# pmcbride/denoise-gan

Hardware: AMD Instinct MI355X
Metric: training images/sec, pix2pix 256x256 bs16/GPU (higher is better)
Workload: dtype fp32 (GEMMs fp16x3, operands 2^-22); 1 GPU; pix2pix train_step (train_pix2pix.py:33-71): G(x)+G(y) identity pass, D real+fake, GAN/L1/L2/TV/identity losses, D and G gradients, Keras Adam G and D; VGG19 content loss (seeded stand-in weights: ImageNet weights are a download); model=pix2pix U-Net G (54.4M) + PatchGAN D (2.77M), global_batch=16, batch_per_gpu=16, image_size=256, scale=1, parallelism=dp1, hip_graph=True, identity_pass=True

## Files before the change

### denoise-gan_amd/csrc/conv_tiles.h

```cpp
#pragma once

#define DG_TILES_FP32(X)                                                                         \
    X(0, 128, 128, 2, 2, 32, 2, 1, 2, 1.00)                                                      \
    X(1, 128, 64, 2, 2, 32, 2, 1, 2, 1.12)                                                       \
    X(2, 64, 128, 2, 2, 32, 2, 1, 2, 1.12)                                                       \
    X(3, 64, 64, 2, 2, 32, 2, 1, 3, 1.35)                                                        \
    X(4, 32, 128, 1, 4, 32, 2, 1, 3, 1.50)                                                       \
    X(5, 128, 128, 2, 2, 16, 3, 1, 3, 1.00)                                                      \
    X(6, 128, 64, 2, 2, 16, 3, 1, 3, 1.12)                                                       \
    X(7, 128, 32, 4, 1, 32, 2, 1, 3, 1.40)                                                       \
    X(8, 256, 32, 4, 1, 32, 2, 1, 2, 1.30)

#define DG_TILES_F16_BK 32
#define DG_TILES_X6(X)                                                                           \
    X(0, 128, 128, 2, 2, 16, 2, 3, 2, 1.00)                                                      \
    X(1, 128, 64, 2, 2, 16, 2, 3, 2, 1.15)                                                       \
    X(2, 64, 128, 2, 2, 16, 2, 3, 2, 1.15)                                                       \
    X(3, 64, 64, 2, 2, 16, 3, 3, 4, 1.40)                                                        \
    X(4, 256, 128, 4, 2, 16, 2, 3, 1, 1.00)                                                      \
    X(5, 128, 256, 2, 4, 16, 2, 3, 1, 0.90)                                                      \
    X(6, 128, 32, 4, 1, 16, 3, 3, 4, 1.45)

#ifndef DG_X3_NB0
#define DG_X3_NB0 2
#endif
#ifndef DG_X3_NB12
#define DG_X3_NB12 2
#endif
#define DG_TILES_X3(X)                                                                           \
    X(0, 128, 128, 2, 2, 32, 2, DG_X3_NB0, 2, 1.00)                                              \
    X(1, 128, 64, 2, 2, 32, 2, DG_X3_NB12, 3, 1.15)                                              \
    X(2, 64, 128, 2, 2, 32, 2, DG_X3_NB12, 3, 1.15)                                              \
    X(3, 64, 64, 2, 2, 32, 3, 3, 3, 1.40)                                                        \
    X(4, 256, 128, 4, 2, 32, 1, 2, 1, 1.00)                                                      \
    X(5, 128, 256, 2, 4, 32, 1, 2, 1, 0.90)                                                      \
    X(6, 128, 32, 4, 1, 32, 3, 3, 2, 1.45)
```

### denoise-gan_amd/csrc/conv_x6.hip

```cpp
#include "conv_x6.h"
#include "conv_tiles.h"
#include <algorithm>

namespace dg {

__global__ void __launch_bounds__(256)
k_split3(const float *__restrict__ src, int ld, long rows, int C, unsigned short *__restrict__ dst) {
    const int C8 = C >> 3;
    const long total = rows * C8;
    const bool vec = ((ld & 3) == 0) && ((((uintptr_t)src) & 15) == 0);
    for (long e = (long)blockIdx.x * blockDim.x + threadIdx.x; e < total; e += (long)gridDim.x * blockDim.x) {
        const long r = e / C8;
        const int c = (int)(e - r * C8) * 8;
        const float *sp = src + r * ld + c;
        f32x4 v0, v1;
        if (vec) {
            v0 = *reinterpret_cast<const f32x4 *>(sp);
            v1 = *reinterpret_cast<const f32x4 *>(sp + 4);
        } else {
            v0 = f32x4{sp[0], sp[1], sp[2], sp[3]};
            v1 = f32x4{sp[4], sp[5], sp[6], sp[7]};
        }
        unsigned h0, m0, l0, h1, m1, l1, h2, m2, l2, h3, m3, l3;
        split3(v0[0], v0[1], h0, m0, l0);
        split3(v0[2], v0[3], h1, m1, l1);
        split3(v1[0], v1[1], h2, m2, l2);
        split3(v1[2], v1[3], h3, m3, l3);
        unsigned short *d = dst + r * 3 * C + (c >> 4) * 48 + (c & 8);
        *reinterpret_cast<u32x4 *>(d) = u32x4{h0, h1, h2, h3};
        *reinterpret_cast<u32x4 *>(d + 16) = u32x4{m0, m1, m2, m3};
        *reinterpret_cast<u32x4 *>(d + 32) = u32x4{l0, l1, l2, l3};
    }
}

__global__ void __launch_bounds__(256)
k_split_f16(const float *__restrict__ src, int ld, long rows, int C, _Float16 *__restrict__ dst) {
    const int C8 = C >> 3;
    const long total = rows * C8;
    const bool vec = ((ld & 3) == 0) && ((((uintptr_t)src) & 15) == 0);
    for (long e = (long)blockIdx.x * blockDim.x + threadIdx.x; e < total; e += (long)gridDim.x * blockDim.x) {
        const long r = e / C8;
        const int c = (int)(e - r * C8) * 8;
        const float *sp = src + r * ld + c;
        f32x4 v0, v1;
        if (vec) {
            v0 = *reinterpret_cast<const f32x4 *>(sp);
            v1 = *reinterpret_cast<const f32x4 *>(sp + 4);
        } else {
            v0 = f32x4{sp[0], sp[1], sp[2], sp[3]};
            v1 = f32x4{sp[4], sp[5], sp[6], sp[7]};
        }
        f16x8 h;
#pragma unroll
        for (int q = 0; q < 4; ++q) { h[q] = (_Float16)v0[q]; h[4 + q] = (_Float16)v1[q]; }
        *reinterpret_cast<f16x8 *>(dst + r * C + c) = h;
    }
}

template <int MODE, int BM, int BN, int WGM, int WGN, int MINW, int NBUF = 3, int NI = 3>
__global__ void __launch_bounds__(64 * WGM * WGN, MINW)
k_conv_gemm_x6(const GemmArgs p) {
    static_assert(NBUF >= 2 && NBUF <= 4, "2 to 4 LDS buffers (1 to 3 K-tiles in flight)");
    static_assert(NI == 3 || NI == 2 || NI == 4, "bf16x6 (3 plane images), fp16 (2 chunk images), fp16x3 (4)");
    constexpr bool X6 = NI == 3;
    constexpr bool X3 = NI == 4;
    constexpr int BK = X6 ? 16 : 32;
    constexpr int GS = 16 * NI;
    constexpr int RM = X6 ? 3 : (X3 ? 2 : 1);
    constexpr bool A_KC = (MODE != MODE_WGRAD);
    constexpr bool B_KC = (MODE == MODE_DGRAD);
    constexpr int NT = 64 * WGM * WGN;
    constexpr int WTM = BM / WGM, WTN = BN / WGN;
    constexpr int TM = WTM / 16, TN = WTN / 16;
    constexpr int APL = BM * 32 + 96, BPL = BN * 32 + 96;
    constexpr int BUF = NI * (APL + BPL);
    constexpr int NW_ = WGM * WGN;
    static_assert(WGM * WGN == 4 || WGM * WGN == 8, "4 or 8 waves");
    static_assert(TM >= 1 && TN >= 1 && WTM % 16 == 0 && WTN % 16 == 0, "wave tile of 16x16 tiles");
    static_assert(BM % 32 == 0 && BN % 32 == 0 && BM <= 256 && BN <= 256, "tile");

    constexpr int STAGE = 16 * (WTN + 4);
    constexpr int BUF0 = BUF > NW_ * STAGE * 4 ? BUF : NW_ * STAGE * 4;
    __shared__ __attribute__((aligned(16))) char smem0[BUF0];
    __shared__ __attribute__((aligned(16))) char smem1[BUF];
    __shared__ __attribute__((aligned(16))) char smem2[NBUF >= 3 ? BUF : 16];
    __shared__ __attribute__((aligned(16))) char smem3[NBUF == 4 ? BUF : 16];

    const ConvGeom &g = p.g;
    const int tid = threadIdx.x;
    const int lane = tid & 63;
    const int wid = __builtin_amdgcn_readfirstlane(tid >> 6);
    const int wm = wid / WGN, wn = wid % WGN;
    const int l32 = lane & 31, h2 = lane >> 5;
    X3Pre x3s;
    if constexpr (X3) x3s = x3_pre(p);

    int zz, tile;
    xcd_remap(zz, tile);
    const int phase = zz / p.splits;
    const int split = zz - phase * p.splits;
    const int mt = tile / p.ntiles;
    const int nt = tile - mt * p.ntiles;
    const int m0 = mt * BM, n0 = nt * BN;

    int Mrows = p.M;
    PhaseInfo ph{};
    if constexpr (MODE == MODE_DGRAD) {
        ph = phase_info(g, phase, g.N);
        Mrows = ph.Mp;
        if (m0 >= Mrows) return;
    }
    const int kbeg = split * p.kchunk;
    const int kend = min(p.K, kbeg + p.kchunk);
    if (kbeg >= kend) return;
    const int nk = (kend - kbeg + BK - 1) / BK;

    constexpr int NW = WGM * WGN;
    constexpr int A_SL = NI * BM / 32, B_SL = NI * BN / 32;
    constexpr int A_NJ = (A_SL + NW - 1) / NW, B_NJ = (B_SL + NW - 1) / NW;
    struct Slot { int plane, r, c; bool live; };
    auto slot_of = [&](int d, bool kc, int X) __attribute__((always_inline)) {
        Slot sl; const int per = X / 32;
        sl.plane = d / per;
        const int pos = (d - sl.plane * per) * 1024 + 16 * lane;
        if (kc) {
            sl.r = pos >> 5;
            sl.c = (pos >> 4) & 1;
        } else {
            sl.r = pos / (2 * X);
            const int pdw = (pos - sl.r * 2 * X) >> 2;
            sl.c = 2 * (pdw ^ x6_rc_swz_cols(X, sl.r));
        }
        return sl;
    };
    Slot asl[A_NJ], bsl[B_NJ];
#pragma unroll
    for (int j = 0; j < A_NJ; ++j) {
        const int d = wid + NW * j;
        asl[j] = slot_of(d < A_SL ? d : 0, A_KC, BM);
        asl[j].live = d < A_SL;
    }
#pragma unroll
    for (int j = 0; j < B_NJ; ++j) {
        const int d = wid + NW * j;
        bsl[j] = slot_of(d < B_SL ? d : 0, B_KC, BN);
        bsl[j].live = d < B_SL;
    }
    constexpr bool A_ALL = (A_SL % NW) == 0, B_ALL = (B_SL % NW) == 0;
    constexpr int NMINE = A_NJ + B_NJ;

    int arow_n[A_NJ], arow_h[A_NJ], arow_w[A_NJ];
    int wg_i[A_NJ], wg_j[A_NJ], wg_ci[A_NJ];
#pragma unroll
    for (int j = 0; j < A_NJ; ++j) {
        arow_n[j] = -1; arow_h[j] = 0; arow_w[j] = 0; wg_i[j] = 0; wg_j[j] = 0; wg_ci[j] = 0;
        if constexpr (A_KC) {
            int m = m0 + asl[j].r;
            if (m < Mrows) {
                if constexpr (MODE == MODE_FWD) {
                    int wo = m % g.Wo; int t = m / g.Wo; int ho = t % g.Ho; int n = t / g.Ho;
                    arow_n[j] = n; arow_h[j] = ho * g.sh - g.pt; arow_w[j] = wo * g.sw - g.pl;
                } else {
                    int ww = m % ph.Wp; int t = m / ph.Wp; int hh = t % ph.Hp; int n = t / ph.Hp;
                    arow_n[j] = n;
                    arow_h[j] = hh + (ph.ph + g.pt - ph.i0h) / g.sh;
                    arow_w[j] = ww + (ph.pw + g.pl - ph.i0w) / g.sw;
                }
            }
        } else {
            int mc = m0 + asl[j].c;
            if (mc < p.M) {
                arow_n[j] = 0;
                int tap = mc / g.Ci; int ci = mc - tap * g.Ci; wg_i[j] = tap / g.kw; wg_j[j] = tap - wg_i[j] * g.kw;
                wg_ci[j] = X6 ? (ci >> 4) * 48 + 16 * asl[j].plane + (ci & 8)
                              : (X3 ? (ci >> 5) * 64 + 32 * (asl[j].plane >> 1) + (ci & 31) : ci);
            }
        }
    }

    const int TA = MODE == MODE_FWD ? g.kh : g.Th, TB = MODE == MODE_FWD ? g.kw : g.Tw;
    int wk_a = 0, wk_b = 0, wk_chunk = 0;
    if constexpr (MODE != MODE_WGRAD) {
        int kk = kbeg / BK; wk_chunk = kk / (TA * TB); int t = kk - wk_chunk * TA * TB;
        wk_a = t / TB; wk_b = t - wk_a * TB;
    }
    int abase[A_NJ], amask[A_NJ], bbase[B_NJ];
    bool bok[B_NJ];
    if constexpr (MODE != MODE_WGRAD) {
#pragma unroll
        for (int j = 0; j < A_NJ; ++j) {
            abase[j] = 0; amask[j] = 0;
            if (arow_n[j] < 0) continue;
            if constexpr (MODE == MODE_FWD) {
                abase[j] = (((arow_n[j] * g.H + arow_h[j]) * g.W + arow_w[j]) * (RM * p.lda) + 16 * asl[j].plane +
                            8 * asl[j].c) * 2;
                for (int a = 0; a < TA; ++a)
                    for (int b = 0; b < TB; ++b) {
                        const int hi = arow_h[j] + a, wi = arow_w[j] + b;
                        if ((unsigned)hi < (unsigned)g.H && (unsigned)wi < (unsigned)g.W) amask[j] |= 1 << (a * TB + b);
                    }
            } else {
                abase[j] = (((arow_n[j] * g.Ho + arow_h[j]) * g.Wo + arow_w[j]) * (RM * p.lda) + 16 * asl[j].plane +
                            8 * asl[j].c) * 2;
                for (int a = 0; a < TA; ++a)
                    for (int b = 0; b < TB; ++b) {
                        const int i = ph.i0h + a * g.sh, jj = ph.i0w + b * g.sw;
                        const int ho = arow_h[j] - a, wo = arow_w[j] - b;
                        if (i < g.kh && jj < g.kw && (unsigned)ho < (unsigned)g.Ho && (unsigned)wo < (unsigned)g.Wo)
                            amask[j] |= 1 << (a * TB + b);
                    }
            }
        }
#pragma unroll
        for (int j = 0; j < B_NJ; ++j) {
            if constexpr (MODE == MODE_FWD) {
                const int col = n0 + bsl[j].c;
                bok[j] = col < p.N;
                bbase[j] = X6 ? (bsl[j].r * (3 * p.ldb) + (col >> 4) * 48 + 16 * bsl[j].plane + (col & 8)) * 2
                         : X3 ? ((bsl[j].r + 16 * (bsl[j].plane & 1)) * (2 * p.ldb) + (col >> 4) * 32 +
                                 16 * (bsl[j].plane >> 1) + (col & 8)) * 2
                              : ((bsl[j].r + 16 * bsl[j].plane) * p.ldb + col) * 2;
            } else {
                const int ci = n0 + bsl[j].r;
                bok[j] = ci < p.N;
                bbase[j] = (ci * (RM * p.ldb) + 16 * bsl[j].plane + 8 * bsl[j].c) * 2;
            }
        }
    }
    auto walk_next = [&]() __attribute__((always_inline)) {
        const int nb = wk_b + 1;
        const bool wb = nb == TB;
        const int na = wk_a + (wb ? 1 : 0);
        const bool wa = na == TA;
        wk_b = wb ? 0 : nb;
        wk_a = wa ? 0 : na;
        wk_chunk += wa ? 1 : 0;
    };

    const rsrc4_t rA = make_rsrc4(p.A, p.a_bytes);
    const rsrc4_t rB = make_rsrc4(p.B, p.b_bytes);
    auto dma = [](rsrc4_t r, char *lds_base, unsigned off) __attribute__((always_inline)) { dma16(r, lds_base, off); };
    auto fdiv = [](unsigned n, unsigned mul, int shr) __attribute__((always_inline)) { return (__umulhi(n, mul) + n) >> shr; };

    auto issue_tile = [&](int k0, char *sm) __attribute__((always_inline)) {
        char *As = sm;
        char *Bs = As + NI * APL;
        int a_delta = 0, b_delta = 0, tap_bit = 0;
        bool b_tap_ok = true;
        if constexpr (MODE == MODE_FWD) {
            a_delta = ((wk_a * g.W + wk_b) * (RM * p.lda) + wk_chunk * GS) * 2;
            b_delta = (((wk_a * g.kw + wk_b) * g.Ci + wk_chunk * BK) * (RM * p.ldb)) * 2;
            tap_bit = wk_a * TB + wk_b;
        } else if constexpr (MODE == MODE_DGRAD) {
            a_delta = (wk_chunk * GS - (wk_a * g.Wo + wk_b) * (RM * p.lda)) * 2;
            const int i = ph.i0h + wk_a * g.sh, jj = ph.i0w + wk_b * g.sw;
            b_tap_ok = i < g.kh && jj < g.kw;
            b_delta = ((b_tap_ok ? (i * g.kw + jj) * g.Ci * (RM * p.ldb) : 0) + wk_chunk * GS) * 2;
            tap_bit = wk_a * TB + wk_b;
        }
        (void)a_delta; (void)b_delta; (void)tap_bit; (void)b_tap_ok;
        const bool live = MODE == MODE_WGRAD || k0 < kend;
#pragma unroll
        for (int j = 0; j < A_NJ; ++j) {
            const int d = asl[j].live ? wid + NW * j : 0, per = BM / 32;
            char *dst = As + asl[j].plane * APL + (d - asl[j].plane * per) * 1024;
            unsigned off;
            bool ok;
            if constexpr (MODE != MODE_WGRAD) {
                ok = (amask[j] >> tap_bit) & 1;
                off = (unsigned)(abase[j] + a_delta);
            } else {
                const unsigned pix = (unsigned)(k0 + asl[j].r + (X6 ? 0 : 16 * (X3 ? asl[j].plane & 1 : asl[j].plane)));
                const unsigned t = fdiv(pix, p.mg_wo, p.sh_wo); const int wo = (int)(pix - t * g.Wo);
                const unsigned n = fdiv(t, p.mg_ho, p.sh_ho); const int ho = (int)(t - n * g.Ho);
                const int hi = ho * g.sh - g.pt + wg_i[j], wi = wo * g.sw - g.pl + wg_j[j];
                ok = arow_n[j] >= 0 && (int)pix < kend && (unsigned)hi < (unsigned)g.H && (unsigned)wi < (unsigned)g.W;
                off = ((unsigned)(((int)n * g.H + hi) * g.W + wi) * (RM * p.lda) + wg_ci[j]) * 2u;
            }
            dma(rA, dst, ok && live ? off : DG_OOB);
        }
#pragma unroll
        for (int j = 0; j < B_NJ; ++j) {
            const int d = bsl[j].live ? wid + NW * j : 0, per = BN / 32;
            char *dst = Bs + bsl[j].plane * BPL + (d - bsl[j].plane * per) * 1024;
            unsigned off;
            bool ok;
            if constexpr (MODE == MODE_FWD) {
                ok = bok[j];
                off = (unsigned)(bbase[j] + b_delta);
            } else if constexpr (MODE == MODE_DGRAD) {
                ok = bok[j] && b_tap_ok;
                off = (unsigned)(bbase[j] + b_delta);
            } else {
                const int col = n0 + bsl[j].c;
                const int pix = k0 + bsl[j].r + (X6 ? 0 : 16 * (X3 ? bsl[j].plane & 1 : bsl[j].plane));
                ok = col < p.N && pix < kend;
                off = X6 ? ((unsigned)pix * (3 * p.ldb) + (col >> 4) * 48 + 16 * bsl[j].plane + (col & 8)) * 2u
                    : X3 ? ((unsigned)pix * (2 * p.ldb) + (col >> 5) * 64 + 32 * (bsl[j].plane >> 1) + (col & 31)) * 2u
                         : ((unsigned)pix * p.ldb + col) * 2u;
            }
            dma(rB, dst, ok && live ? off : DG_OOB);
        }
        if constexpr (MODE != MODE_WGRAD) walk_next();
    };
    auto barrier = []() __attribute__((always_inline)) {
        asm volatile("s_waitcnt lgkmcnt(0)" ::: "memory");
        __builtin_amdgcn_s_barrier();
        asm volatile("" ::: "memory");
    };

    f32x4 acc[TM][TN];
#pragma unroll
    for (int a = 0; a < TM; ++a)
#pragma unroll
        for (int b = 0; b < TN; ++b) acc[a][b] = f32x4{0.f, 0.f, 0.f, 0.f};

    auto frag = [&](const char *p0, const char *p1, int rc0, bool kc, bool is_a) __attribute__((always_inline)) {
        if (kc) return x6_kc_frag(p0, p1, rc0, lane);
        return is_a ? x6_rc_frag<BM>(p0, p1, rc0, lane) : x6_rc_frag<BN>(p0, p1, rc0, lane);
    };
    auto read_frags = [&](const char *sm, bf16x8 (&ahm)[TM], bf16x8 (&ahl)[TM], bf16x8 (&b1)[TN],
                          bf16x8 (&b2)[TN], bf16x8 (&b3)[TN]) __attribute__((always_inline)) {
        const char *A0 = sm, *A1 = sm + APL, *A2 = sm + (NI - 1) * APL;
        const char *B0 = sm + NI * APL, *B1 = B0 + BPL, *B2 = B0 + (NI - 1) * BPL;
#pragma unroll
        for (int a = 0; a < TM; ++a) {
            const int r0 = wm * WTM + a * 16;
            ahm[a] = frag(A0, A1, r0, A_KC, true);
            if constexpr (X6) ahl[a] = frag(A0, A2, r0, A_KC, true);
        }
#pragma unroll
        for (int b = 0; b < TN; ++b) {
            const int c0 = wn * WTN + b * 16;
            b1[b] = frag(B0, B1, c0, B_KC, false);
            if constexpr (X6) {
                b2[b] = frag(B1, B0, c0, B_KC, false);
                b3[b] = frag(B2, B0, c0, B_KC, false);
            }
        }
    };

    constexpr int AHEAD = NBUF - 1;
#if defined(DG_NO_MIDB)
    constexpr bool MIDB = false;
#elif defined(DG_MIDB_X3)
    constexpr bool MIDB = X3;
#else
    constexpr bool MIDB = true;
#endif
    constexpr int DIST = MIDB ? NBUF : AHEAD;
    auto ktile = [&](int kt, const char *cur, char *nxt) __attribute__((always_inline)) {
        if constexpr (X3) {
            f16x8 ah[TM], al[TM], bh[TN], bl[TN];
            const char *B0 = cur + 4 * APL;
#pragma unroll
            for (int a = 0; a < TM; ++a) {
                const int r0 = wm * WTM + a * 16;
                ah[a] = __builtin_bit_cast(f16x8, frag(cur, cur + APL, r0, A_KC, true));
                al[a] = __builtin_bit_cast(f16x8, frag(cur + 2 * APL, cur + 3 * APL, r0, A_KC, true));
            }
            constexpr int BH1 = B_KC ? 2 : 1, BL0 = B_KC ? 1 : 2;
#pragma unroll
            for (int b = 0; b < TN; ++b) {
                const int c0 = wn * WTN + b * 16;
                bh[b] = __builtin_bit_cast(f16x8, frag(B0, B0 + BH1 * BPL, c0, B_KC, false));
                bl[b] = __builtin_bit_cast(f16x8, frag(B0 + BL0 * BPL, B0 + 3 * BPL, c0, B_KC, false));
            }
            if constexpr (MIDB) {
                barrier();
                issue_tile(kbeg + (kt + DIST) * BK, const_cast<char *>(cur));
            } else {
                issue_tile(kbeg + (kt + AHEAD) * BK, nxt);
            }
#pragma unroll
            for (int a = 0; a < TM; ++a)
#pragma unroll
                for (int b = 0; b < TN; ++b)
                    acc[a][b] = __builtin_amdgcn_mfma_f32_16x16x32_f16(ah[a], bh[b], acc[a][b], 0, 0, 0);
#pragma unroll
            for (int a = 0; a < TM; ++a)
#pragma unroll
                for (int b = 0; b < TN; ++b)
                    acc[a][b] = __builtin_amdgcn_mfma_f32_16x16x32_f16(al[a], bh[b], acc[a][b], 0, 0, 0);
#pragma unroll
            for (int a = 0; a < TM; ++a)
#pragma unroll
                for (int b = 0; b < TN; ++b)
                    acc[a][b] = __builtin_amdgcn_mfma_f32_16x16x32_f16(ah[a], bl[b], acc[a][b], 0, 0, 0);
            wait_dma_c<(DIST - 1) * NMINE>();
            barrier();
            return;
        }
        bf16x8 ahm[TM], ahl[X6 ? TM : 1], b1[TN], b2[X6 ? TN : 1], b3[X6 ? TN : 1];
        if constexpr (X6) {
            read_frags(cur, ahm, ahl, b1, b2, b3);
        } else {
            bf16x8 dA[TM], dB[TN];
            read_frags(cur, ahm, dA, b1, dB, dB);
        }
        if constexpr (MIDB) {
            barrier();
            issue_tile(kbeg + (kt + DIST) * BK, const_cast<char *>(cur));
        } else {
            issue_tile(kbeg + (kt + AHEAD) * BK, nxt);
        }
        if constexpr (X6) {
#pragma unroll
            for (int a = 0; a < TM; ++a)
#pragma unroll
                for (int b = 0; b < TN; ++b)
                    acc[a][b] = __builtin_amdgcn_mfma_f32_16x16x32_bf16(ahm[a], b1[b], acc[a][b], 0, 0, 0);
#pragma unroll
            for (int a = 0; a < TM; ++a)
#pragma unroll
                for (int b = 0; b < TN; ++b)
                    acc[a][b] = __builtin_amdgcn_mfma_f32_16x16x32_bf16(ahm[a], b2[b], acc[a][b], 0, 0, 0);
#pragma unroll
            for (int a = 0; a < TM; ++a)
#pragma unroll
                for (int b = 0; b < TN; ++b)
                    acc[a][b] = __builtin_amdgcn_mfma_f32_16x16x32_bf16(ahl[a], b3[b], acc[a][b], 0, 0, 0);
        } else {
#pragma unroll
            for (int a = 0; a < TM; ++a)
#pragma unroll
                for (int b = 0; b < TN; ++b)
                    acc[a][b] = __builtin_amdgcn_mfma_f32_16x16x32_f16(__builtin_bit_cast(f16x8, ahm[a]),
                                                                       __builtin_bit_cast(f16x8, b1[b]), acc[a][b],
                                                                       0, 0, 0);
        }
        wait_dma_c<(DIST - 1) * NMINE>();
        barrier();
    };
    auto pipeline = [&](char *L0, char *L1, char *L2, char *L3) __attribute__((always_inline)) {
        issue_tile(kbeg, L0);
        if constexpr (DIST >= 2) issue_tile(kbeg + BK, L1);
        if constexpr (DIST >= 3) issue_tile(kbeg + 2 * BK, L2);
        if constexpr (DIST >= 4) issue_tile(kbeg + 3 * BK, L3);
        wait_dma_c<(DIST - 1) * NMINE>();
        barrier();
        int kt = 0;
        if constexpr (NBUF == 2) {
            for (; kt + 1 < nk; kt += 2) {
                ktile(kt, L0, L1);
                ktile(kt + 1, L1, L0);
            }
            if (kt < nk) ktile(kt, L0, L1);
        } else if constexpr (NBUF == 3) {
            for (; kt + 2 < nk; kt += 3) {
                ktile(kt, L0, L2);
                ktile(kt + 1, L1, L0);
                ktile(kt + 2, L2, L1);
            }
            if (kt < nk) ktile(kt, L0, L2);
            if (kt + 1 < nk) ktile(kt + 1, L1, L0);
        } else {
            for (; kt + 3 < nk; kt += 4) {
                ktile(kt, L0, L3);
                ktile(kt + 1, L1, L0);
                ktile(kt + 2, L2, L1);
                ktile(kt + 3, L3, L2);
            }
            if (kt < nk) ktile(kt, L0, L3);
            if (kt + 1 < nk) ktile(kt + 1, L1, L0);
            if (kt + 2 < nk) ktile(kt + 2, L2, L1);
        }
    };
    pipeline(smem0, smem1, smem2, smem3);

    wait_dma_c<0>();
    barrier();
    float ys_pre = 0.f;
    if constexpr (X3) {
        const float osc = x3_out_scale(p, x3s);
        ys_pre = p.yp ? x3_raw_scale(x3s.y, F16X3_XS) : 0.f;
#pragma unroll
        for (int a = 0; a < TM; ++a)
#pragma unroll
            for (int b = 0; b < TN; ++b) acc[a][b] *= osc;
    }
    static_assert(NW * STAGE * 4 <= BUF0, "epilogue staging fits in LDS buffer 0");
    const bool ident = MODE != MODE_DGRAD || (g.sh == 1 && g.sw == 1);
    auto rowmap = [&](int row) __attribute__((always_inline)) -> RowPix {
        if (row >= Mrows) return RowPix{-1, -1};
        long pix = row;
        if constexpr (MODE == MODE_DGRAD) {
            if (!ident && p.splits == 1) {
                int ww = row % ph.Wp; int t = row / ph.Wp; int hh = t % ph.Hp; int n = t / ph.Hp;
                pix = (long)(n * g.H + hh * g.sh + ph.ph) * g.W + ww * g.sw + ph.pw;
            }
        }
        return RowPix{row, pix};
    };
    conv_epilogue16<MODE, TM, TN>(p, acc, m0 + wm * WTM, n0 + wn * WTN, rowmap, phase, split, lane,
                                  reinterpret_cast<float *>(smem0) + wid * STAGE, ys_pre);
}

void launch_split3(const float *src, int ld, long rows, int C, unsigned short *dst, hipStream_t s) {
    const long total = rows * (C / 8);
    if (total == 0) return;
    const unsigned blocks = (unsigned)std::min<long>((total + 255) / 256, 8192);
    hipLaunchKernelGGL(k_split3, dim3(blocks), dim3(256), 0, s, src, ld, rows, C, dst);
}

template <int G>
__global__ void __launch_bounds__(256)
k_split_x3(const float *__restrict__ src, int ld, long rows, int C, float scale, const float *sm, const float *sg,
           const float *sc, _Float16 *__restrict__ dst) {
    if (sm) scale = x3_grad_scale(sm, sg, sc);
    const int C8 = C >> 3;
    const long total = rows * C8;
    const bool vec = ((ld & 3) == 0) && ((((uintptr_t)src) & 15) == 0);
    for (long e = (long)blockIdx.x * blockDim.x + threadIdx.x; e < total; e += (long)gridDim.x * blockDim.x) {
        const long r = e / C8;
        const int c = (int)(e - r * C8) * 8;
        const float *sp = src + r * ld + c;
        f32x4 v0, v1;
        if (vec) {
            v0 = *reinterpret_cast<const f32x4 *>(sp);
            v1 = *reinterpret_cast<const f32x4 *>(sp + 4);
        } else {
            v0 = f32x4{sp[0], sp[1], sp[2], sp[3]};
            v1 = f32x4{sp[4], sp[5], sp[6], sp[7]};
        }
        f16x8 h, l;
#pragma unroll
        for (int q = 0; q < 4; ++q) {
            _Float16 a, b;
            split_x3(v0[q], scale, a, b);
            h[q] = a; l[q] = b;
            split_x3(v1[q], scale, a, b);
            h[4 + q] = a; l[4 + q] = b;
        }
        _Float16 *d = dst + r * 2 * C + (c / G) * (2 * G) + (c % G);
        *reinterpret_cast<f16x8 *>(d) = h;
        *reinterpret_cast<f16x8 *>(d + G) = l;
    }
}

void launch_split_x3(const float *src, int ld, long rows, int C, void *dst, int group, float scale, hipStream_t s,
                     const float *sm, const float *sg, const float *sc) {
    const long total = rows * (C / 8);
    if (total == 0) return;
    const unsigned blocks = (unsigned)std::min<long>((total + 255) / 256, 8192);
    if (group == 32)
        hipLaunchKernelGGL(k_split_x3<32>, dim3(blocks), dim3(256), 0, s, src, ld, rows, C, scale, sm, sg, sc,
                           (_Float16 *)dst);
    else
        hipLaunchKernelGGL(k_split_x3<16>, dim3(blocks), dim3(256), 0, s, src, ld, rows, C, scale, sm, sg, sc,
                           (_Float16 *)dst);
}

__global__ void __launch_bounds__(256) k_absmax(const float *__restrict__ x, long rows, int C, int ld, float *out) {
    float m = 0.f;
    const long total = rows * C;
    if (ld == C && ((((uintptr_t)x) & 15) == 0)) {
        const long t4 = total >> 2;
        const long st = (long)gridDim.x * blockDim.x;
        long e = (long)blockIdx.x * blockDim.x + threadIdx.x;
        auto m4 = [](f32x4 v) { return fmaxf(fmaxf(fabsf(v[0]), fabsf(v[1])), fmaxf(fabsf(v[2]), fabsf(v[3]))); };
        for (; e + 3 * st < t4; e += 4 * st) {
            f32x4 v[4];
#pragma unroll
            for (int u = 0; u < 4; ++u) v[u] = reinterpret_cast<const f32x4 *>(x)[e + u * st];
#pragma unroll
            for (int u = 0; u < 4; ++u) m = fmaxf(m, m4(v[u]));
        }
        for (; e < t4; e += st) m = fmaxf(m, m4(reinterpret_cast<const f32x4 *>(x)[e]));
        for (long e = (t4 << 2) + (long)blockIdx.x * blockDim.x + threadIdx.x; e < total;
             e += (long)gridDim.x * blockDim.x)
            m = fmaxf(m, fabsf(x[e]));
    } else {
        for (long e = (long)blockIdx.x * blockDim.x + threadIdx.x; e < total; e += (long)gridDim.x * blockDim.x) {
            const long r = e / C;
            m = fmaxf(m, fabsf(x[r * ld + (e - r * C)]));
        }
    }
    block_atomic_absmax(out, m);
}

__global__ void __launch_bounds__(256) k_weight_bound(const float *__restrict__ w, long K, int Co,
                                                     const float *__restrict__ bias, float *gout, float *cout,
                                                     float *zero8) {
    __shared__ float red[256];
    if (zero8 && threadIdx.x < X3_SHARDS) zero8[threadIdx.x * X3_SHARD_STRIDE] = 0.f;
    const int cl = threadIdx.x & 63, rl = threadIdx.x >> 6;
    float g = 0.f, c = 0.f;
    for (int c0 = 0; c0 < Co; c0 += 64) {
        const int co = c0 + cl;
        float sum = 0.f;
        if (co < Co) {
            long k = rl;
            for (; k + 28 < K; k += 32) {
                float v[8];
#pragma unroll
                for (int u = 0; u < 8; ++u) v[u] = w[(k + 4 * u) * Co + co];
#pragma unroll
                for (int u = 0; u < 8; ++u) sum += fabsf(v[u]);
            }
            for (; k < K; k += 4) sum += fabsf(w[k * Co + co]);
            if (bias && rl == 0) c = fmaxf(c, fabsf(bias[co]));
        }
        red[threadIdx.x] = sum;
        __syncthreads();
        if (rl == 0) g = fmaxf(g, red[cl] + red[64 + cl] + red[128 + cl] + red[192 + cl]);
        __syncthreads();
    }
    red[threadIdx.x] = g;
    __syncthreads();
    if (threadIdx.x == 0) {
        for (int i = 1; i < 64; ++i) g = fmaxf(g, red[i]);
        gout[0] = g;
    }
    __syncthreads();
    red[threadIdx.x] = c;
    __syncthreads();
    if (threadIdx.x == 0 && cout) {
        for (int i = 1; i < 64; ++i) c = fmaxf(c, red[i]);
        cout[0] = c;
    }
}

__global__ void __launch_bounds__(256) k_weight_bound_cols(const float *__restrict__ w, long K, int Co,
                                                          const float *__restrict__ bias, float *gout, float *cout,
                                                          float *zero8) {
    __shared__ float red[256];
    if (blockIdx.x == 0 && zero8 && threadIdx.x < X3_SHARDS) zero8[threadIdx.x * X3_SHARD_STRIDE] = 0.f;
    const int cl = threadIdx.x & 15, rl = threadIdx.x >> 4;
    const int co = blockIdx.x * 16 + cl;
    float sum = 0.f;
    if (co < Co) {
        long k = rl;
        for (; k + 48 < K; k += 64) {
            float v[4];
#pragma unroll
            for (int u = 0; u < 4; ++u) v[u] = w[(k + 16 * u) * Co + co];
#pragma unroll
            for (int u = 0; u < 4; ++u) sum += fabsf(v[u]);
        }
        for (; k < K; k += 16) sum += fabsf(w[k * Co + co]);
    }
    red[threadIdx.x] = sum;
    __syncthreads();
    if (threadIdx.x < 16) {
        float s = 0.f;
        for (int r = 0; r < 16; ++r) s += red[16 * r + threadIdx.x];
        red[threadIdx.x] = s;
    }
    __syncthreads();
    if (threadIdx.x == 0) {
        float g = 0.f;
        for (int i = 0; i < 16; ++i) g = fmaxf(g, red[i]);
        atomicMax(reinterpret_cast<unsigned *>(gout), __float_as_uint(g));
        if (blockIdx.x == 0 && cout) {
            float c = 0.f;
            if (bias)
                for (int i = 0; i < Co; ++i) c = fmaxf(c, fabsf(bias[i]));
            cout[0] = c;
        }
    }
}

__global__ void __launch_bounds__(256) k_weight_bound_in(const float *__restrict__ w, int taps, int Ci, int Co,
                                                        float *gout) {
    __shared__ float red[256];
    const int ci = blockIdx.x;
    float s = 0.f;
    for (int t = 0; t < taps; ++t) {
        const float *row = w + ((long)t * Ci + ci) * Co;
        for (int co = threadIdx.x; co < Co; co += 256) s += fabsf(row[co]);
    }
    red[threadIdx.x] = s;
    __syncthreads();
#pragma unroll
    for (int h = 128; h > 0; h >>= 1) {
        if (threadIdx.x < h) red[threadIdx.x] += red[threadIdx.x + h];
        __syncthreads();
    }
    if (threadIdx.x == 0) atomicMax(reinterpret_cast<unsigned *>(gout), __float_as_uint(red[0]));
}

constexpr long WBOUND_ONE_BLOCK_MAX = 1 << 16;

void launch_weight_bound(const float *w, long K, int Co, const float *bias, float *gout, float *cout, hipStream_t s,
                         float *zero8) {
    if (K * Co <= WBOUND_ONE_BLOCK_MAX) {
        hipLaunchKernelGGL(k_weight_bound, dim3(1), dim3(256), 0, s, w, K, Co, bias, gout, cout, zero8);
        return;
    }
    hipMemsetAsync(gout, 0, sizeof(float), s);
    hipLaunchKernelGGL(k_weight_bound_cols, dim3((Co + 15) / 16), dim3(256), 0, s, w, K, Co, bias, gout, cout, zero8);
}

void launch_weight_bound_in(const float *w, int taps, int Ci, int Co, float *gout, hipStream_t s) {
    hipMemsetAsync(gout, 0, sizeof(float), s);
    hipLaunchKernelGGL(k_weight_bound_in, dim3(Ci), dim3(256), 0, s, w, taps, Ci, Co, gout);
}

void launch_absmax(const float *x, long rows, int C, int ld, float *out, hipStream_t s) {
    const long total = rows * C;
    if (total == 0) return;
    const unsigned blocks = (unsigned)std::min<long>((total + 255) / 256, 1024);
    hipLaunchKernelGGL(k_absmax, dim3(blocks), dim3(256), 0, s, x, rows, C, ld, out);
}

struct F16Split {
    const float *src;
    int ld;
    long rows;
    int C;
    _Float16 *dst;
};
__global__ void __launch_bounds__(256) k_split_f16_pair(F16Split a, F16Split b, unsigned nba) {
    const bool first = blockIdx.x < nba;
    const F16Split d = first ? a : b;
    const unsigned bid = first ? blockIdx.x : blockIdx.x - nba, nb = first ? nba : gridDim.x - nba;
    const int C8 = d.C >> 3;
    const long total = d.rows * C8;
    const bool vec = ((d.ld & 3) == 0) && ((((uintptr_t)d.src) & 15) == 0);
    for (long e = (long)bid * blockDim.x + threadIdx.x; e < total; e += (long)nb * blockDim.x) {
        const long r = e / C8;
        const int c = (int)(e - r * C8) * 8;
        const float *sp = d.src + r * d.ld + c;
        f32x4 v0, v1;
        if (vec) {
            v0 = *reinterpret_cast<const f32x4 *>(sp);
            v1 = *reinterpret_cast<const f32x4 *>(sp + 4);
        } else {
            v0 = f32x4{sp[0], sp[1], sp[2], sp[3]};
            v1 = f32x4{sp[4], sp[5], sp[6], sp[7]};
        }
        f16x8 h;
#pragma unroll
        for (int q = 0; q < 4; ++q) { h[q] = (_Float16)v0[q]; h[4 + q] = (_Float16)v1[q]; }
        *reinterpret_cast<f16x8 *>(d.dst + r * d.C + c) = h;
    }
}

void launch_split_f16_pair(const float *a, int lda, long ra, int ca, void *da, const float *b, int ldb, long rb,
                           int cb, void *db, hipStream_t s) {
    const long ta = ra * (ca / 8), tb = rb * (cb / 8);
    const unsigned nba = (unsigned)std::max<long>(1, std::min<long>((ta + 255) / 256, 4096));
    const unsigned nbb = (unsigned)std::max<long>(1, std::min<long>((tb + 255) / 256, 4096));
    hipLaunchKernelGGL(k_split_f16_pair, dim3(nba + nbb), dim3(256), 0, s, F16Split{a, lda, ra, ca, (_Float16 *)da},
                       F16Split{b, ldb, rb, cb, (_Float16 *)db}, nba);
}

void launch_split_f16(const float *src, int ld, long rows, int C, void *dst, hipStream_t s) {
    const long total = rows * (C / 8);
    if (total == 0) return;
    const unsigned blocks = (unsigned)std::min<long>((total + 255) / 256, 8192);
    hipLaunchKernelGGL(k_split_f16, dim3(blocks), dim3(256), 0, s, src, ld, rows, C, (_Float16 *)dst);
}

template <int NI>
static int launch_gemm_planes(int mode, int cfg, dim3 grid, const GemmArgs &a, hipStream_t s) {
#define DG_X6(C, BM_, BN_, WM_, WN_, BK_, MW_, NB_, BPC_, EFF_)                                                 \
    case C: {                                                                                                   \
        const dim3 blk(64 * WM_ * WN_);                                                                         \
        if (mode == MODE_FWD) hipLaunchKernelGGL((k_conv_gemm_x6<MODE_FWD, BM_, BN_, WM_, WN_, MW_, NB_, NI>), grid, blk, 0, s, a); \
        else if (mode == MODE_DGRAD) hipLaunchKernelGGL((k_conv_gemm_x6<MODE_DGRAD, BM_, BN_, WM_, WN_, MW_, NB_, NI>), grid, blk, 0, s, a); \
        else hipLaunchKernelGGL((k_conv_gemm_x6<MODE_WGRAD, BM_, BN_, WM_, WN_, MW_, NB_, NI>), grid, blk, 0, s, a); \
        return DG_OK;                                                                                           \
    }
    switch (cfg) {
        DG_TILES_X6(DG_X6)
    default:
        set_error("%s conv GEMM: no tile config %d", NI == 2 ? "fp16" : "bf16x6", cfg);
        return DG_ERR_ARG;
    }
#undef DG_X6
}

int launch_gemm_x6(int mode, int cfg, dim3 grid, const GemmArgs &a, hipStream_t s) {
    return launch_gemm_planes<3>(mode, cfg, grid, a, s);
}

int launch_gemm_f16(int mode, int cfg, dim3 grid, const GemmArgs &a, hipStream_t s) {
    return launch_gemm_planes<2>(mode, cfg, grid, a, s);
}

int launch_gemm_x3(int mode, int cfg, dim3 grid, const GemmArgs &a, hipStream_t s) {
#define DG_X3(C, BM_, BN_, WM_, WN_, BK_, MW_, NB_, BPC_, EFF_)                                                 \
    case C: {                                                                                                   \
        const dim3 blk(64 * WM_ * WN_);                                                                         \
        if (mode == MODE_FWD) hipLaunchKernelGGL((k_conv_gemm_x6<MODE_FWD, BM_, BN_, WM_, WN_, MW_, NB_, 4>), grid, blk, 0, s, a); \
        else if (mode == MODE_DGRAD) hipLaunchKernelGGL((k_conv_gemm_x6<MODE_DGRAD, BM_, BN_, WM_, WN_, MW_, NB_, 4>), grid, blk, 0, s, a); \
        else hipLaunchKernelGGL((k_conv_gemm_x6<MODE_WGRAD, BM_, BN_, WM_, WN_, MW_, NB_, 4>), grid, blk, 0, s, a); \
        return DG_OK;                                                                                           \
    }
    switch (cfg) {
        DG_TILES_X3(DG_X3)
    default:
        set_error("fp16x3 conv GEMM: no tile config %d", cfg);
        return DG_ERR_ARG;
    }
#undef DG_X3
}

}
```

Before: 1040 images/s.

## Add staggered two-half pipeline for 8-wave fp16x3 conv GEMM tiles

For the fp16x3 conv GEMM with 8-wave tiles (256x128 and 128x256), adds a new main loop on three LDS buffers in which the two 4-wave halves are offset by one barrier. Each half then issues MFMAs while the other waits on DMA and LDS reads. Address computation for the next tile is split from the DMA issue, WGRAD A-offsets are reused across slots, and sched_group_barrier hints interleave LDS reads with MFMAs. This costs an extra LDS buffer per block, which may reduce occupancy, and it depends on the mismatched barrier counts between the halves being correct.

```diff
diff --git a/denoise-gan_amd/csrc/conv_tiles.h b/denoise-gan_amd/csrc/conv_tiles.h
--- a/denoise-gan_amd/csrc/conv_tiles.h
+++ b/denoise-gan_amd/csrc/conv_tiles.h
@@ -21,6 +21,13 @@
     X(5, 128, 256, 2, 4, 16, 2, 3, 1, 0.90)                                                      \
     X(6, 128, 32, 4, 1, 16, 3, 3, 4, 1.45)
 
+#ifndef DG_X3_NB45
+#ifdef DG_X3_W8_LOCKSTEP
+#define DG_X3_NB45 2
+#else
+#define DG_X3_NB45 3
+#endif
+#endif
 #ifndef DG_X3_NB0
 #define DG_X3_NB0 2
 #endif
@@ -32,6 +39,6 @@
     X(1, 128, 64, 2, 2, 32, 2, DG_X3_NB12, 3, 1.15)                                              \
     X(2, 64, 128, 2, 2, 32, 2, DG_X3_NB12, 3, 1.15)                                              \
     X(3, 64, 64, 2, 2, 32, 3, 3, 3, 1.40)                                                        \
-    X(4, 256, 128, 4, 2, 32, 1, 2, 1, 1.00)                                                      \
-    X(5, 128, 256, 2, 4, 32, 1, 2, 1, 0.90)                                                      \
+    X(4, 256, 128, 4, 2, 32, 1, DG_X3_NB45, 1, 1.00)                                             \
+    X(5, 128, 256, 2, 4, 32, 1, DG_X3_NB45, 1, 0.90)                                             \
     X(6, 128, 32, 4, 1, 32, 3, 3, 2, 1.45)
diff --git a/denoise-gan_amd/csrc/conv_x6.hip b/denoise-gan_amd/csrc/conv_x6.hip
--- a/denoise-gan_amd/csrc/conv_x6.hip
+++ b/denoise-gan_amd/csrc/conv_x6.hip
@@ -1,6 +1,7 @@
 #include "conv_x6.h"
 #include "conv_tiles.h"
 #include <algorithm>
+#include <type_traits>
 
 namespace dg {
 
@@ -76,6 +77,12 @@
     constexpr int BUF = NI * (APL + BPL);
     constexpr int NW_ = WGM * WGN;
     static_assert(WGM * WGN == 4 || WGM * WGN == 8, "4 or 8 waves");
+#ifdef DG_X3_W8_LOCKSTEP
+    constexpr bool W8 = false;
+#else
+    constexpr bool W8 = X3 && NW_ == 8;
+    static_assert(!W8 || NBUF == 3, "the two-half loop runs on three LDS buffers");
+#endif
     static_assert(TM >= 1 && TN >= 1 && WTM % 16 == 0 && WTN % 16 == 0, "wave tile of 16x16 tiles");
     static_assert(BM % 32 == 0 && BN % 32 == 0 && BM <= 256 && BN <= 256, "tile");
 
@@ -242,7 +249,8 @@
     auto dma = [](rsrc4_t r, char *lds_base, unsigned off) __attribute__((always_inline)) { dma16(r, lds_base, off); };
     auto fdiv = [](unsigned n, unsigned mul, int shr) __attribute__((always_inline)) { return (__umulhi(n, mul) + n) >> shr; };
 
-    auto issue_tile = [&](int k0, char *sm) __attribute__((always_inline)) {
+    auto issue_phase = [&](int k0, char *sm, auto phc, unsigned *o) __attribute__((always_inline)) {
+        constexpr int PH = decltype(phc)::value;
         char *As = sm;
         char *Bs = As + NI * APL;
         int a_delta = 0, b_delta = 0, tap_bit = 0;
@@ -260,6 +268,10 @@
         }
         (void)a_delta; (void)b_delta; (void)tap_bit; (void)b_tap_ok;
         const bool live = MODE == MODE_WGRAD || k0 < kend;
+        constexpr int WSH = (W8 && MODE == MODE_WGRAD && A_ALL && NW % (BM / 32) == 0)
+                                ? ((NW / (BM / 32)) % 2 == 0 ? 1 : 2) : 0;
+        unsigned aoff[A_NJ];
+        bool aok[A_NJ];
 #pragma unroll
         for (int j = 0; j < A_NJ; ++j) {
             const int d = asl[j].live ? wid + NW * j : 0, per = BM / 32;
@@ -269,6 +281,9 @@
             if constexpr (MODE != MODE_WGRAD) {
                 ok = (amask[j] >> tap_bit) & 1;
                 off = (unsigned)(abase[j] + a_delta);
+            } else if (WSH > 0 && j >= WSH) {
+                ok = aok[j - WSH];
+                off = aoff[j - WSH] + 2u * (unsigned)(wg_ci[j] - wg_ci[j - WSH]);
             } else {
                 const unsigned pix = (unsigned)(k0 + asl[j].r + (X6 ? 0 : 16 * (X3 ? asl[j].plane & 1 : asl[j].plane)));
                 const unsigned t = fdiv(pix, p.mg_wo, p.sh_wo); const int wo = (int)(pix - t * g.Wo);
@@ -277,7 +292,10 @@
                 ok = arow_n[j] >= 0 && (int)pix < kend && (unsigned)hi < (unsigned)g.H && (unsigned)wi < (unsigned)g.W;
                 off = ((unsigned)(((int)n * g.H + hi) * g.W + wi) * (RM * p.lda) + wg_ci[j]) * 2u;
             }
-            dma(rA, dst, ok && live ? off : DG_OOB);
+            aok[j] = ok; aoff[j] = off;
+            if constexpr (PH == 0) dma(rA, dst, ok && live ? off : DG_OOB);
+            else if constexpr (PH == 1) o[j] = ok && live ? off : DG_OOB;
+            else dma(rA, dst, o[j]);
         }
 #pragma unroll
         for (int j = 0; j < B_NJ; ++j) {
@@ -299,9 +317,14 @@
                     : X3 ? ((unsigned)pix * (2 * p.ldb) + (col >> 5) * 64 + 32 * (bsl[j].plane >> 1) + (col & 31)) * 2u
                          : ((unsigned)pix * p.ldb + col) * 2u;
             }
-            dma(rB, dst, ok && live ? off : DG_OOB);
-        }
-        if constexpr (MODE != MODE_WGRAD) walk_next();
+            if constexpr (PH == 0) dma(rB, dst, ok && live ? off : DG_OOB);
+            else if constexpr (PH == 1) o[A_NJ + j] = ok && live ? off : DG_OOB;
+            else dma(rB, dst, o[A_NJ + j]);
+        }
+        if constexpr (MODE != MODE_WGRAD && PH != 2) walk_next();
+    };
+    auto issue_tile = [&](int k0, char *sm) __attribute__((always_inline)) {
+        issue_phase(k0, sm, std::integral_constant<int, 0>{}, nullptr);
     };
     auto barrier = []() __attribute__((always_inline)) {
         asm volatile("s_waitcnt lgkmcnt(0)" ::: "memory");
@@ -349,44 +372,79 @@
     constexpr bool MIDB = true;
 #endif
     constexpr int DIST = MIDB ? NBUF : AHEAD;
+#ifndef DG_X3_ABL
+#define DG_X3_ABL 0
+#endif
+    constexpr int ABL = (X3 && NW_ == 8) ? DG_X3_ABL : 0;
+    auto x3_read = [&](const char *cur, f16x8 (&ah)[TM], f16x8 (&al)[TM], f16x8 (&bh)[TN],
+                       f16x8 (&bl)[TN]) __attribute__((always_inline)) {
+        if constexpr ((ABL & 4) != 0) {
+#pragma unroll
+            for (int a = 0; a < TM; ++a) asm volatile("" : "=v"(ah[a]), "=v"(al[a]));
+#pragma unroll
+            for (int b = 0; b < TN; ++b) asm volatile("" : "=v"(bh[b]), "=v"(bl[b]));
+            return;
+        }
+        const char *B0 = cur + 4 * APL;
+#pragma unroll
+        for (int a = 0; a < TM; ++a) {
+            const int r0 = wm * WTM + a * 16;
+            ah[a] = __builtin_bit_cast(f16x8, frag(cur, cur + APL, r0, A_KC, true));
+            al[a] = __builtin_bit_cast(f16x8, frag(cur + 2 * APL, cur + 3 * APL, r0, A_KC, true));
+        }
+        constexpr int BH1 = B_KC ? 2 : 1, BL0 = B_KC ? 1 : 2;
+#pragma unroll
+        for (int b = 0; b < TN; ++b) {
+            const int c0 = wn * WTN + b * 16;
+            bh[b] = __builtin_bit_cast(f16x8, frag(B0, B0 + BH1 * BPL, c0, B_KC, false));
+            bl[b] = __builtin_bit_cast(f16x8, frag(B0 + BL0 * BPL, B0 + 3 * BPL, c0, B_KC, false));
+        }
+    };
+    auto x3_mfma = [&](const f16x8 (&ah)[TM], const f16x8 (&al)[TM], const f16x8 (&bh)[TN],
+                       const f16x8 (&bl)[TN]) __attribute__((always_inline)) {
+        if constexpr ((ABL & 1) != 0) {
+#pragma unroll
+            for (int a = 0; a < TM; ++a) asm volatile("" ::"v"(ah[a]), "v"(al[a]));
+#pragma unroll
+            for (int b = 0; b < TN; ++b) asm volatile("" ::"v"(bh[b]), "v"(bl[b]));
+            return;
+        }
+#pragma unroll
+        for (int a = 0; a < TM; ++a)
+#pragma unroll
+            for (int b = 0; b < TN; ++b)
+                acc[a][b] = __builtin_amdgcn_mfma_f32_16x16x32_f16(ah[a], bh[b], acc[a][b], 0, 0, 0);
+#pragma unroll
+        for (int a = 0; a < TM; ++a)
+#pragma unroll
+            for (int b = 0; b < TN; ++b)
+                acc[a][b] = __builtin_amdgcn_mfma_f32_16x16x32_f16(al[a], bh[b], acc[a][b], 0, 0, 0);
+#pragma unroll
+        for (int a = 0; a < TM; ++a)
+#pragma unroll
+            for (int b = 0; b < TN; ++b)
+                acc[a][b] = __builtin_amdgcn_mfma_f32_16x16x32_f16(ah[a], bl[b], acc[a][b], 0, 0, 0);
+    };
+    auto x3_issue = [&](int k0, char *sm) __attribute__((always_inline)) {
+        if constexpr ((ABL & 2) == 0) issue_tile(k0, sm);
+    };
+    auto x3_offs = [&](int k0, unsigned (&o)[NMINE]) __attribute__((always_inline)) {
+        if constexpr ((ABL & 2) == 0) issue_phase(k0, nullptr, std::integral_constant<int, 1>{}, o);
+    };
+    auto x3_fire = [&](char *sm, unsigned (&o)[NMINE]) __attribute__((always_inline)) {
+        if constexpr ((ABL & 2) == 0) issue_phase(0, sm, std::integral_constant<int, 2>{}, o);
+    };
     auto ktile = [&](int kt, const char *cur, char *nxt) __attribute__((always_inline)) {
         if constexpr (X3) {
             f16x8 ah[TM], al[TM], bh[TN], bl[TN];
-            const char *B0 = cur + 4 * APL;
-#pragma unroll
-            for (int a = 0; a < TM; ++a) {
-                const int r0 = wm * WTM + a * 16;
-                ah[a] = __builtin_bit_cast(f16x8, frag(cur, cur + APL, r0, A_KC, true));
-                al[a] = __builtin_bit_cast(f16x8, frag(cur + 2 * APL, cur + 3 * APL, r0, A_KC, true));
-            }
-            constexpr int BH1 = B_KC ? 2 : 1, BL0 = B_KC ? 1 : 2;
-#pragma unroll
-            for (int b = 0; b < TN; ++b) {
-                const int c0 = wn * WTN + b * 16;
-                bh[b] = __builtin_bit_cast(f16x8, frag(B0, B0 + BH1 * BPL, c0, B_KC, false));
-                bl[b] = __builtin_bit_cast(f16x8, frag(B0 + BL0 * BPL, B0 + 3 * BPL, c0, B_KC, false));
-            }
+            x3_read(cur, ah, al, bh, bl);
             if constexpr (MIDB) {
                 barrier();
-                issue_tile(kbeg + (kt + DIST) * BK, const_cast<char *>(cur));
+                x3_issue(kbeg + (kt + DIST) * BK, const_cast<char *>(cur));
             } else {
-                issue_tile(kbeg + (kt + AHEAD) * BK, nxt);
-            }
-#pragma unroll
-            for (int a = 0; a < TM; ++a)
-#pragma unroll
-                for (int b = 0; b < TN; ++b)
-                    acc[a][b] = __builtin_amdgcn_mfma_f32_16x16x32_f16(ah[a], bh[b], acc[a][b], 0, 0, 0);
-#pragma unroll
-            for (int a = 0; a < TM; ++a)
-#pragma unroll
-                for (int b = 0; b < TN; ++b)
-                    acc[a][b] = __builtin_amdgcn_mfma_f32_16x16x32_f16(al[a], bh[b], acc[a][b], 0, 0, 0);
-#pragma unroll
-            for (int a = 0; a < TM; ++a)
-#pragma unroll
-                for (int b = 0; b < TN; ++b)
-                    acc[a][b] = __builtin_amdgcn_mfma_f32_16x16x32_f16(ah[a], bl[b], acc[a][b], 0, 0, 0);
+                x3_issue(kbeg + (kt + AHEAD) * BK, nxt);
+            }
+            x3_mfma(ah, al, bh, bl);
             wait_dma_c<(DIST - 1) * NMINE>();
             barrier();
             return;
@@ -432,11 +490,54 @@
         wait_dma_c<(DIST - 1) * NMINE>();
         barrier();
     };
+    auto ktile_w8 = [&](int kt, const char *cur, char *nxt, unsigned (&o)[NMINE]) __attribute__((always_inline)) {
+        x3_fire(nxt, o);
+        __builtin_amdgcn_sched_barrier(0);
+        f16x8 ah[TM], al[TM], bh[TN], bl[TN];
+        x3_read(cur, ah, al, bh, bl);
+        wait_dma_c<NMINE>();
+        barrier();
+        __builtin_amdgcn_sched_barrier(0);
+        x3_offs(kbeg + (kt + 3) * BK, o);
+        x3_mfma(ah, al, bh, bl);
+#pragma unroll
+        for (int i = 0; i < 16; ++i) __builtin_amdgcn_sched_group_barrier(0x008, 1, 0);
+#pragma unroll
+        for (int i = 0; i < 32; ++i) {
+            __builtin_amdgcn_sched_group_barrier(0x006, 3, 0);
+            __builtin_amdgcn_sched_group_barrier(0x008, 1, 0);
+        }
+        __builtin_amdgcn_sched_barrier(0);
+        barrier();
+    };
+    auto pipeline_w8 = [&](char *L0, char *L1, char *L2) __attribute__((always_inline)) {
+        const int half = wid >> 2;
+        unsigned o[NMINE] = {};
+        x3_issue(kbeg, L0);
+        x3_issue(kbeg + BK, L1);
+        x3_offs(kbeg + 2 * BK, o);
+        wait_dma_c<NMINE>();
+        barrier();
+        if (half) barrier();
+        int kt = 0;
+        for (; kt + 2 < nk; kt += 3) {
+            ktile_w8(kt, L0, L2, o);
+            ktile_w8(kt + 1, L1, L0, o);
+            ktile_w8(kt + 2, L2, L1, o);
+        }
+        if (kt < nk) ktile_w8(kt, L0, L2, o);
+        if (kt + 1 < nk) ktile_w8(kt + 1, L1, L0, o);
+        if (!half) barrier();
+    };
     auto pipeline = [&](char *L0, char *L1, char *L2, char *L3) __attribute__((always_inline)) {
-        issue_tile(kbeg, L0);
-        if constexpr (DIST >= 2) issue_tile(kbeg + BK, L1);
-        if constexpr (DIST >= 3) issue_tile(kbeg + 2 * BK, L2);
-        if constexpr (DIST >= 4) issue_tile(kbeg + 3 * BK, L3);
+        if constexpr (W8) {
+            pipeline_w8(L0, L1, L2);
+            return;
+        }
+        x3_issue(kbeg, L0);
+        if constexpr (DIST >= 2) x3_issue(kbeg + BK, L1);
+        if constexpr (DIST >= 3) x3_issue(kbeg + 2 * BK, L2);
+        if constexpr (DIST >= 4) x3_issue(kbeg + 3 * BK, L3);
         wait_dma_c<(DIST - 1) * NMINE>();
         barrier();
         int kt = 0;
```

Result: faster. 1063 images/s (median of 6 runs) (+2.2%).
